# ToyotaResearchInstitute/conex

Measured on AMD Instinct MI355X. Metric: Newton KKT-solves/sec (assemble+factor+solve), 1000x(20x20) PSD blocks, fp64, higher is better.
Workload: dtype f64

## Files before the change

conex_amd/csrc/dense_elim.hip.h:

```cpp
#pragma once
#include "device_utils.h"

namespace cxk {

__device__ __forceinline__ void SqrtAndInverse(double d, double& root, double& inv) {
  const double r0 = __builtin_amdgcn_rsq(d);
  double g = d * r0, h = 0.5 * r0;
  double e = fma(-h, g, 0.5);
  g = fma(g, e, g);
  h = fma(h, e, h);
  e = fma(-h, g, 0.5);
  g = fma(g, e, g);
  h = fma(h, e, h);
  const double res = fma(-g, g, d);
  root = fma(res, h, g);
  inv = h + h;
}

template <int LEN, int C0, int C1, int BASE>
struct DppColumns {
  static __device__ __forceinline__ void run(double (&a)[LEN], double w, double v) {
    if constexpr (C0 < C1) {
      asm("v_fmac_f64_dpp %0, %1, %2 row_newbcast:%3 row_mask:0xf bank_mask:0xf"
          : "+v"(a[C0])
          : "v"(w), "v"(v), "n"(C0 - BASE));
      DppColumns<LEN, C0 + 1, C1, BASE>::run(a, w, v);
    }
  }
};

__device__ __forceinline__ void DppOperandFence(double& x, double& y, double& z) {
  asm("s_nop 1" : "+v"(x), "+v"(y), "+v"(z));
}


template <int NSMAX, int SMAX, int J, int C, int LEN>
__device__ __forceinline__ void ElimFmac(double (&a)[LEN], double x0, double x1) {
  if constexpr (C < 16) {
    asm volatile("v_fmac_f64_dpp %0, %1, -%2 row_newbcast:%3 row_mask:0xf bank_mask:0xf"
                 : "+v"(a[C])
                 : "v"(x0), "v"(a[J]), "n"(C));
  } else if constexpr (NSMAX == 16) {
    asm volatile("v_fmac_f64_dpp %0, %1, -%1 row_newbcast:%2 row_mask:0xf bank_mask:0xf"
                 : "+v"(a[C])
                 : "v"(a[J]), "n"(C - 16));
  } else {
    asm volatile("v_fmac_f64_dpp %0, %1, -%2 row_newbcast:%3 row_mask:0xf bank_mask:0xf"
                 : "+v"(a[C])
                 : "v"(x1), "v"(a[J]), "n"(C - 16));
  }
}

template <int NSMAX, int SMAX, int J, int P0, int CNT, int N, int LEN>
__device__ __forceinline__ void ElimIssue(double (&a)[LEN], double x0, double x1) {
  if constexpr (CNT > 0 && P0 < N) {
    ElimFmac<NSMAX, SMAX, J, J + 1 + P0>(a, x0, x1);
    ElimIssue<NSMAX, SMAX, J, P0 + 1, CNT - 1, N>(a, x0, x1);
  }
}

__device__ __forceinline__ int OpaqueLane(int lane) {
  int z;
  asm volatile("s_mov_b32 %0, 0" : "=s"(z));
  return lane + z;
}

template <int J>
__device__ __forceinline__ double ElimPivotColumn(double v, int lz, unsigned long long& m, double& s0, double& s1) {
  typedef unsigned u2 __attribute__((ext_vector_type(2)));
  __builtin_amdgcn_sched_barrier(0);
  m = __builtin_amdgcn_ballot_w64(lz == J);
  asm volatile("" : : "s"(m));
  __builtin_amdgcn_sched_barrier(0);
  double c0, c1;
  asm volatile("v_mov_b64 %0, %2\n\tv_mov_b64 %1, %2" : "=&v"(c0), "=&v"(c1) : "v"(v));
  __builtin_amdgcn_sched_barrier(0);
  const double d = ReadLane(v, J);
  __builtin_amdgcn_sched_barrier(0);
  const u2 l = __builtin_amdgcn_permlane16_swap(__double2loint(c0), __double2loint(c1), false, false);
  const u2 h = __builtin_amdgcn_permlane16_swap(__double2hiint(c0), __double2hiint(c1), false, false);
  s0 = __hiloint2double(h.x, l.x);
  s1 = __hiloint2double(h.y, l.y);
  __builtin_amdgcn_sched_barrier(0);
  return d;
}

template <int NSMAX, int SMAX, int J, int NRHS = 1, bool CHECK = true>
struct ElimSteps {
  static constexpr int LEN = NSMAX + SMAX + NRHS, RB = NSMAX + SMAX;
  static __device__ __forceinline__ void run(double (&a)[LEN], int lane, bool& bad, int ns) {
    if constexpr (J == 0 && NSMAX > 0) {
      if constexpr (kPipelined) {
        unsigned long long m;
        double s0, s1;
        const int lz = OpaqueLane(lane);
        const double d = ElimPivotColumn<0>(a[0], lz, m, s0, s1);
        if constexpr (CHECK) bad |= !(d > 0.0);
        double root, inv;
        SqrtAndInverse(d, root, inv);
        step(a, lane, bad, root, inv, ns, lz, m, s0, s1);
      } else {
        const double d = ReadLane(a[0], 0);
        if constexpr (CHECK) bad |= !(d > 0.0);
        double root, inv;
        SqrtAndInverse(d, root, inv);
        step(a, lane, bad, root, inv, ns);
      }
    }
  }
  static constexpr bool kPipelined = NSMAX + SMAX > 16 && NSMAX + SMAX <= 32;
  static __device__ __forceinline__ void step(double (&a)[LEN], int lane, bool& bad, double root, double inv, int ns,
                                              int lz = 0, unsigned long long m = 0, double s0 = 0.0, double s1 = 0.0) {
    if constexpr (kPipelined && J < NSMAX) {
      if (J >= ns) return;
      constexpr int N = NSMAX + SMAX - J - 1;
      const double x0 = s0 * inv, x1 = s1 * inv, t = a[J] * inv;
      __builtin_amdgcn_sched_barrier(0);
      a[J] = __builtin_amdgcn_inverse_ballot_w64(m) ? root : t;
      __builtin_amdgcn_sched_barrier(0);
      if constexpr (NSMAX == 16 && J + 1 >= 16 && N > 0) asm volatile("s_nop 1");
      ElimIssue<NSMAX, SMAX, J, 0, 1, N>(a, x0, x1);
      double root1 = 1.0, inv1 = 1.0, t0 = 0.0, t1 = 0.0;
      unsigned long long m1 = 0;
      if constexpr (J + 1 < NSMAX) {
        const double d1 = ElimPivotColumn<J + 1>(a[J + 1], lz, m1, t0, t1);
        if constexpr (CHECK) bad |= !(d1 > 0.0);
#define CXK_ELIM_FILL(P0, CNT)                      \
  __builtin_amdgcn_sched_barrier(0);                \
  ElimIssue<NSMAX, SMAX, J, P0, CNT, N>(a, x0, x1); \
  __builtin_amdgcn_sched_barrier(0)
        const double r0 = __builtin_amdgcn_rsq(d1);
        CXK_ELIM_FILL(1, 2);
        double g = d1 * r0, hh = 0.5 * r0;
        CXK_ELIM_FILL(3, 2);
        double e = fma(-hh, g, 0.5);
        CXK_ELIM_FILL(5, 2);
        g = fma(g, e, g);
        hh = fma(hh, e, hh);
        CXK_ELIM_FILL(7, 2);
        e = fma(-hh, g, 0.5);
        CXK_ELIM_FILL(9, 2);
        g = fma(g, e, g);
        hh = fma(hh, e, hh);
        CXK_ELIM_FILL(11, 2);
        const double res = fma(-g, g, d1);
        inv1 = hh + hh;
        CXK_ELIM_FILL(13, 2);
        root1 = fma(res, hh, g);
        CXK_ELIM_FILL(15, 64);
#undef CXK_ELIM_FILL
        asm volatile("" : : "v"(root1), "v"(inv1));
      } else {
        ElimIssue<NSMAX, SMAX, J, 1, 64, N>(a, x0, x1);
        __builtin_amdgcn_sched_barrier(0);
      }
#pragma unroll
      for (int q = 0; q < NRHS; q++) {
        const double yj = ReadLane(a[RB + q], J) * inv;
        if (lane > J)
          a[RB + q] = fma(-yj, a[J], a[RB + q]);
        else if (lane == J)
          a[RB + q] = yj;
      }
      ElimSteps<NSMAX, SMAX, J + 1, NRHS, CHECK>::step(a, lane, bad, root1, inv1, ns, lz, m1, t0, t1);
    } else if constexpr (J < NSMAX) {
      if (J >= ns) return;
      a[J] = (lane == J) ? root : a[J] * inv;
      double root1 = 1.0, inv1 = 1.0;
      auto next_pivot = [&]() {
        if constexpr (J + 1 < NSMAX) {
          const double d1 = ReadLane(a[J + 1], J + 1);
          if constexpr (CHECK) bad |= !(d1 > 0.0);
          SqrtAndInverse(d1, root1, inv1);
        }
      };
      if constexpr (NSMAX + SMAX <= 16) {
        double naj = -a[J];
        double dummy = 0.0;
        DppOperandFence(dummy, naj, a[J]);
        DppColumns<LEN, J + 1, (J + 2 < NSMAX + SMAX ? J + 2 : NSMAX + SMAX), 0>::run(a, a[J], naj);
        next_pivot();
        DppColumns<LEN, J + 2, NSMAX + SMAX, 0>::run(a, a[J], naj);
      } else {
        if constexpr (J + 1 < NSMAX + SMAX) a[J + 1] = fma(-ReadLane(a[J], J + 1), a[J], a[J + 1]);
        next_pivot();
#pragma unroll
        for (int c = J + 2; c < NSMAX + SMAX; c++) a[c] = fma(-ReadLane(a[J], c), a[J], a[c]);
      }
#pragma unroll
      for (int q = 0; q < NRHS; q++) {
        const double yj = ReadLane(a[RB + q], J) * inv;
        if (lane > J)
          a[RB + q] = fma(-yj, a[J], a[RB + q]);
        else if (lane == J)
          a[RB + q] = yj;
      }
      ElimSteps<NSMAX, SMAX, J + 1, NRHS, CHECK>::step(a, lane, bad, root1, inv1, ns);
    }
  }
};

}
```

conex_amd/csrc/tree_fused.hip:

```cpp
#include <hip/hip_runtime.h>
#include <hip/hip_ext.h>

#include <type_traits>

#include "tree_supernode.hip.h"
#include "kernels_kkt_top.hip.h"
#include "tree_fused.h"

namespace cxk {

constexpr int kFusedSpinLimit = 1 << 18;

#ifdef CXK_FUSED_STAMPS
constexpr int kFusedStampWaves = 8192;
__device__ long long g_fused_tree_stamp[kFusedStampWaves * 16];
#define FT_STAMP(i) ft_stamp[i] = __builtin_amdgcn_s_memrealtime()
#define FT_COUNT(i, v) ft_stamp[i] = (v)
#define FT_STAMP_DECL long long ft_stamp[16] = {0, 0, 0, 0, 0, 0, 0, 0, 0, 0, 0, 0, 0, 0, 0, 0}
#define FT_STAMP_FLUSH(level)                                                              \
  do {                                                                                     \
    if ((threadIdx.x & 63) == 0 && blockIdx.x < kFusedStampWaves) {                        \
      ft_stamp[15] = (level);                                                              \
      for (int i_ = 0; i_ < 16; i_++) g_fused_tree_stamp[blockIdx.x * 16 + i_] = ft_stamp[i_]; \
    }                                                                                      \
  } while (0)
#else
#define FT_STAMP(i) do { } while (0)
#define FT_COUNT(i, v) do { } while (0)
#define FT_STAMP_DECL do { } while (0)
#define FT_STAMP_FLUSH(level) do { } while (0)
#endif

__device__ __forceinline__ double LoadAgent(const double* p) {
  return __hip_atomic_load(p, __ATOMIC_RELAXED, __HIP_MEMORY_SCOPE_AGENT);
}
__device__ __forceinline__ void StoreAgent(double* p, double v) {
  __hip_atomic_store(p, v, __ATOMIC_RELAXED, __HIP_MEMORY_SCOPE_AGENT);
}
__device__ __forceinline__ bool IsSentinel(double v) {
  return (unsigned long long)__double_as_longlong(v) == kFusedSentinel;
}
__device__ __forceinline__ double SentinelValue() { return __longlong_as_double((long long)kFusedSentinel); }
__device__ __forceinline__ int64_t Join64(int lo, int hi) { return ((int64_t)hi << 32) | (uint32_t)lo; }

__device__ __forceinline__ void SleepUnits(int units) {
  for (; units >= 32; units -= 32) __builtin_amdgcn_s_sleep(32);
  for (; units >= 4; units -= 4) __builtin_amdgcn_s_sleep(4);
}

__device__ __forceinline__ void ReportTimeout(const FusedTreeArgs& A) {
  if ((threadIdx.x & 63) == 0) {
    atomicExch(A.fail + 1, A.tag);
    __hip_atomic_store(A.host_flag, 1.0, __ATOMIC_RELAXED, __HIP_MEMORY_SCOPE_SYSTEM);
  }
}

template <int NC, int PRW>
struct FusedImg {
  unsigned off[NC];
  unsigned aw, bi, o0, sl;
  int pd[PRW];
  unsigned pk[PRW];
};
struct FusedNoImg {};

constexpr int FusedRounds(int smax, int nrhs) { return (smax * (smax + 1) / 2 + nrhs * smax + 63) / 64; }
template <int NA, int SA, int NB, int SB, int NRHS>
struct FusedImgOf {
  static constexpr FusedImgLayout kLy = FusedImgLayoutOf(NA, SA, NB, SB);
  static constexpr int kRa = FusedRounds(SA, NRHS), kRb = FusedRounds(SB, NRHS);
  static constexpr int kRounds = kRa > kRb ? (kRa > 1 ? kRa : 1) : (kRb > 1 ? kRb : 1);
  using type = FusedImg<kLy.nc, kRounds>;
  static_assert(kLy.nc % 4 == 0 && NA + SA < kLy.rows && NB + SB < kLy.rows, "rows of four-word groups, one spare row");
  static __device__ __forceinline__ type Load(const FusedTreeArgs& A, int pos) {
    type I;
    const int lane = threadIdx.x & 63;
    const unsigned* im = A.img + (size_t)pos * kLy.stride;
    const int row = lane < kLy.rows - 1 ? lane : kLy.rows - 1;
    const uint4* po = reinterpret_cast<const uint4*>(im + row * kLy.nc);
#pragma unroll
    for (int q = 0; q < kLy.nc / 4; q++) {
      const uint4 v = po[q];
      I.off[4 * q] = v.x;
      I.off[4 * q + 1] = v.y;
      I.off[4 * q + 2] = v.z;
      I.off[4 * q + 3] = v.w;
    }
    const uint4 l = *reinterpret_cast<const uint4*>(im + kLy.l_at + 4 * row);
    I.aw = l.x;
    I.bi = l.y;
    I.o0 = l.z;
    I.sl = l.w;
#pragma unroll
    for (int r = 0; r < kRounds; r++) {
      const int t = lane + 64 * r;
      const uint2 u = *reinterpret_cast<const uint2*>(im + kLy.u_at + 2 * (t < kLy.ul ? t : 0));
      I.pd[r] = (int)u.x;
      I.pk[r] = u.y;
    }
    return I;
  }
};

template <int J>
__device__ __forceinline__ void FmacRowBcast(double& acc, double w, double v) {
  asm("v_fmac_f64_dpp %0, %1, %2 row_newbcast:%3 row_mask:0xf bank_mask:0xf" : "+v"(acc) : "v"(w), "v"(v), "n"(J));
}

template <int NSMAX, int SMAX, bool UP_ONLY = false, bool FROM_X = false, int NRHS = 1, class IMG = FusedNoImg>
__device__ __forceinline__ void FusedSupernode(const FusedTreeArgs& A, const int w, double* __restrict__ my, const IMG& I = IMG{}) {
  static_assert(NSMAX + SMAX <= 64, "one lane per panel row");
  constexpr bool IMAGED = !std::is_same<IMG, FusedNoImg>::value;
  static_assert(IMAGED == (!FROM_X && NSMAX <= 32), "two-row frames that load from the Schur blocks: the image");
  static_assert(NRHS == 1 || (NRHS == 3 && !UP_ONLY && !FROM_X && NSMAX <= 32), "three right-hand sides: the one-launch sweep of a single GPU");
  constexpr int RB = NSMAX + SMAX, MMAX = NRHS > 1 ? 4 : kFastSlots, MFMAX = MMAX, XMAX = kFusedExtraSlots;
  constexpr int RL = FusedRhsLane(NSMAX, SMAX);
  constexpr bool ROWRHS = RL >= 0 && !UP_ONLY && !FROM_X;
  constexpr int NCOL = ROWRHS ? 0 : NRHS;
  constexpr int NVMAX = SMAX * (SMAX + 1) / 2 + NRHS * SMAX;
  constexpr int PR = (NVMAX + 63) / 64;
  const int lane = threadIdx.x & 63;
  FT_STAMP_DECL;
  FT_STAMP(0);
  FT_COUNT(10, __builtin_amdgcn_s_getreg((31 << 11) | 4));
  FT_COUNT(11, __builtin_amdgcn_s_getreg((31 << 11) | 20));
  const SnRec R = DecodeRec(w);
  FT_STAMP(1);
  auto f = [&](int i) { return __builtin_amdgcn_readlane(w, 32 + i); };
  const int ns = R.ns, s = R.nsep;
  const bool is_row = lane < ns;
  const int sc = lane - NSMAX;
  const bool is_sep = sc >= 0 && sc < s;
  double* base = A.slab + R.diag_off;
  const unsigned rel = (unsigned)(R.offd_off - R.diag_off);
  unsigned o0, st;
  int lim;
  if constexpr (IMAGED) {
    o0 = I.o0;
    st = I.sl & 0xffffu;
    lim = (int)(I.sl >> 16);
  } else {
    o0 = is_row ? (unsigned)lane : (is_sep ? rel + (unsigned)(sc * ns) : 0u);
    st = is_row ? (unsigned)ns : 1u;
    lim = is_row ? lane + 1 : (is_sep ? ns : 0);
  }
  const int gen = A.gen;
  double* handG = A.hand + (int64_t)gen * A.hand_stride;
  double* handO = A.hand + (int64_t)(gen ^ 1) * A.hand_stride;
  double* ysG = A.ysig + (int64_t)gen * A.ysig_stride;
  double* ysO = A.ysig + (int64_t)(gen ^ 1) * A.ysig_stride;
  double* handT = A.hand + (int64_t)A.tgen * A.hand_stride;
  double* handTO = A.hand + (int64_t)(A.tgen ^ 1) * A.hand_stride;
  double* ysT = A.ysig + (int64_t)A.tgen * A.ysig_stride;
  double* ysTO = A.ysig + (int64_t)(A.tgen ^ 1) * A.ysig_stride;
  const int pub_beg = __builtin_amdgcn_readlane(w, 23);
  const int npairs = s * (s + 1) / 2, nv = npairs + NRHS * s;

  double a[NSMAX + SMAX + NCOL];
  double rv[NRHS];
  double fwx = 0.0;
  double awv, aqv;
  double rb;
  int pd[PR > 0 ? PR : 1], prd[PR > 0 ? PR : 1];
  bool pdt[PR > 0 ? PR : 1];
  pd[0] = prd[0] = 0;
  pdt[0] = false;
  if constexpr (IMAGED) {
    const char* gb = reinterpret_cast<const char*>(A.G);
#pragma unroll
    for (int j = 0; j < NSMAX; j++) a[j] = *reinterpret_cast<const double*>(gb + I.off[j]);
    awv = A.AWc[I.aw];
    aqv = A.AQcc[I.aw];
    rb = A.b[I.bi];
#pragma unroll
    for (int r = 0; r < PR; r++) {
      const unsigned pk = ROWRHS ? I.pk[r] : I.pk[r] >> 16;
      pd[r] = I.pd[r];
      prd[r] = (SMAX + NRHS) * (int)(pk & 255u) + (int)((pk >> 8) & 127u);
      pdt[r] = (int)I.pk[r] < 0;
    }
  } else {
  const double* Gk = A.G + (FROM_X ? 0 : Join64(f(0), f(1)));
  const int64_t roff = FROM_X ? 0 : Join64(f(2), f(3));
  const int M = f(4);
  const int q = is_row ? lane : (is_sep ? ns + sc : 0);
  const int mypr = (__builtin_amdgcn_ds_bpermute(4 * (32 + 6 + (q >> 2)), w) >> (8 * (q & 3))) & 255;
  const int myp = mypr == 255 ? 0 : mypr;
  const int has_fill = FROM_X ? 0 : f(5);
  if constexpr (FROM_X) {
    const int64_t xsb = Join64(f(0), f(1));
    const double* xd = A.x + xsb;
    const unsigned tri = (unsigned)(ns * (ns + 1) / 2);
#pragma unroll
    for (int j = 0; j < NSMAX; j++) {
      const unsigned dj = (unsigned)(j * ns - j * (j - 1) / 2);
      const unsigned idx = is_row ? dj + (unsigned)(lane - j) : tri + (unsigned)(sc * ns + j);
      a[j] = xd[(j < lim) ? idx : 0u];
    }
  } else {
    const char* gb = reinterpret_cast<const char*>(Gk);
    const unsigned myp8 = 8u * (unsigned)myp;
#pragma unroll
    for (int j = 0; j < NSMAX; j++) {
      const unsigned pj = (unsigned)((f(6 + (j >> 2)) >> (8 * (j & 3))) & 255);
      const unsigned pj8 = 8u * (pj == 255u ? 0u : pj);
      const unsigned hi8 = myp8 > pj8 ? myp8 : pj8, lo8 = myp8 > pj8 ? pj8 : myp8;
      a[j] = *reinterpret_cast<const double*>(gb + (__umul24(lo8, (unsigned)M) + hi8));
    }
    if (has_fill) {
#pragma unroll
      for (int j = 0; j < NSMAX; j++) {
        const unsigned pj = (unsigned)((f(6 + (j >> 2)) >> (8 * (j & 3))) & 255);
        a[j] = (mypr == 255 || pj == 255u) ? 0.0 : a[j];
      }
    }
  }
  const int pr = is_row ? myp : (f(6) & 255);
  if constexpr (FROM_X) {
    const int64_t xv = A.n_xs + f(2) + (is_row ? lane : 0);
    awv = A.x[xv];
    aqv = A.x[xv + A.n_xv];
    fwx = A.x[xv + 2 * (int64_t)A.n_xv];
  } else {
    awv = A.AWc[roff + pr];
    aqv = A.AQcc[roff + pr];
  }
  rb = A.b[R.start + (is_row ? lane : 0)];
#pragma unroll
  for (int r = 0; r < PR; r++) {
    const int t = lane + 64 * r;
    const int tq = (NRHS > 1 && t >= npairs + s && s > 0) ? (t - npairs) / s : 0;
    const int tk = t - tq * s;
    pdt[r] = tq > 0;
    pd[r] = A.pub[pub_beg + (t < nv ? tk : 0)] + tq * (int)A.fwd_stride;
    int k = 0, rem = t < npairs ? t : 0;
    while (rem >= s - k && k < s) {
      rem -= s - k;
      k++;
    }
    const int kk = t < npairs ? k : tk - npairs, cc = t < npairs ? k + rem : SMAX + tq;
    if (ROWRHS && t >= npairs)
      prd[r] = (SMAX + NRHS) * (RL + (t < nv ? tq : 0)) + (t < nv ? kk : 0);
    else
      prd[r] = (SMAX + NRHS) * (NSMAX + (t < nv ? kk : 0)) + (t < nv ? cc : 0);
  }
  }
  const int ntg = R.tg_end - R.tg_beg;
  int ploc0 = 0, ploc1 = 0;
  if (ntg > 0) {
    ploc0 = A.tg_reg[R.tg_beg + (lane < ntg ? lane : 0)];
    if (ntg > 64) ploc1 = A.tg_reg[R.tg_beg + (lane + 64 < ntg ? lane + 64 : 0)];
  }
  const int xt_beg = f(24), nxt = FROM_X ? 0 : f(25), mx = f(26), rbase = f(27), mr = FROM_X ? 0 : f(28);
  const int64_t xbase = Join64(f(29), f(30));
  int xloc0 = 0, xloc1 = 0;
  double gx0[XMAX], gx1[XMAX];
#pragma unroll
  for (int i = 0; i < XMAX; i++) gx0[i] = gx1[i] = 0.0;
  if (nxt > 0) {
    const int mxl = mx > 0 ? mx - 1 : 0;
    {
      const int ts = lane < nxt ? lane : 0;
      xloc0 = A.xreg[xt_beg + ts];
      long long xs[XMAX];
#pragma unroll
      for (int i = 0; i < XMAX; i++) xs[i] = A.xsrc[xbase + (int64_t)ts * mx + (i < mx ? i : mxl)];
#pragma unroll
      for (int i = 0; i < XMAX; i++) {
        const double v = A.G[xs[i] >= 0 ? xs[i] : 0];
        gx0[i] = (i < mx && xs[i] >= 0 && lane < nxt) ? v : 0.0;
      }
    }
    if (nxt > 64) {
      const int ts = lane + 64 < nxt ? lane + 64 : 0;
      xloc1 = A.xreg[xt_beg + ts];
      long long xs[XMAX];
#pragma unroll
      for (int i = 0; i < XMAX; i++) xs[i] = A.xsrc[xbase + (int64_t)ts * mx + (i < mx ? i : mxl)];
#pragma unroll
      for (int i = 0; i < XMAX; i++) {
        const double v = A.G[xs[i] >= 0 ? xs[i] : 0];
        gx1[i] = (i < mx && xs[i] >= 0 && lane + 64 < nxt) ? v : 0.0;
      }
    }
  }
#pragma unroll
  for (int j = 0; j < NSMAX; j++) a[j] = 0.0 + a[j];
  awv = 0.0 + awv;
  aqv = 0.0 + aqv;
  if (mr > 0) {
    const int mrl = mr - 1;
    long long rs[XMAX];
#pragma unroll
    for (int i = 0; i < XMAX; i++) rs[i] = A.rsrc[rbase + (is_row ? lane : 0) * mr + (i < mr ? i : mrl)];
    double ax[XMAX], qx[XMAX];
#pragma unroll
    for (int i = 0; i < XMAX; i++) {
      ax[i] = A.AWc[rs[i] >= 0 ? rs[i] : 0];
      qx[i] = A.AQcc[rs[i] >= 0 ? rs[i] : 0];
    }
    if (rs[0] >= 0) {
      awv = 0.0;
      aqv = 0.0;
    }
#pragma unroll
    for (int i = 0; i < XMAX; i++)
      if (i < mr && rs[i] >= 0) {
        awv += ax[i];
        aqv += qx[i];
      }
    for (int c0 = XMAX; c0 < mr; c0 += XMAX) {
#pragma unroll
      for (int i = 0; i < XMAX; i++) rs[i] = A.rsrc[rbase + (is_row ? lane : 0) * mr + (c0 + i < mr ? c0 + i : mrl)];
#pragma unroll
      for (int i = 0; i < XMAX; i++) {
        ax[i] = A.AWc[rs[i] >= 0 ? rs[i] : 0];
        qx[i] = A.AQcc[rs[i] >= 0 ? rs[i] : 0];
      }
#pragma unroll
      for (int i = 0; i < XMAX; i++)
        if (c0 + i < mr && rs[i] >= 0) {
          awv += ax[i];
          aqv += qx[i];
        }
    }
  }
  if constexpr (NRHS == 1) {
    if (A.comb)
      rb = A.cb * rb + A.cq * aqv + A.cw * awv;
    else
      rb = A.k * (rb * A.bs + aqv * A.cs) - 2 * awv;
  }
  if constexpr (FROM_X) rb -= fwx;
  if constexpr (!IMAGED) {
#pragma unroll
    for (int j = 0; j < NSMAX; j++) a[j] = (j < lim) ? a[j] : 0.0;
#pragma unroll
    for (int j = 0; j < NSMAX; j++)
      if (j >= ns && lane == j) a[j] = 1.0;
  }
#pragma unroll
  for (int c = 0; c < SMAX; c++) a[NSMAX + c] = 0.0;
  rv[0] = is_row ? (NRHS == 1 ? rb : rb * A.bs) : 0.0;
  if constexpr (NRHS == 3) {
    rv[1] = is_row ? aqv * A.cs : 0.0;
    rv[2] = is_row ? awv : 0.0;
  }
  FT_STAMP(2);

  const bool pulls = ntg > 0 || R.mf > 0;
  if (nxt > 0 || ntg > 0) {
#pragma unroll
    for (int j = 0; j < NSMAX; j++) my[64 * j + lane] = a[j];
    WaveSync();
    if (nxt > 0) {
      if (lane < nxt) {
        double acc = my[xloc0];
#pragma unroll
        for (int i = 0; i < XMAX; i++) acc += gx0[i];
        my[xloc0] = acc;
      }
      if (lane + 64 < nxt) {
        double acc = my[xloc1];
#pragma unroll
        for (int i = 0; i < XMAX; i++) acc += gx1[i];
        my[xloc1] = acc;
      }
      for (int c0 = XMAX; c0 < mx; c0 += XMAX)
        for (int half = 0; half < 2 && 64 * half < nxt; half++) {
          const int t = lane + 64 * half;
          const int ts = t < nxt ? t : 0;
          long long xs[XMAX];
          double gv[XMAX];
#pragma unroll
          for (int i = 0; i < XMAX; i++) xs[i] = A.xsrc[xbase + (int64_t)ts * mx + (c0 + i < mx ? c0 + i : mx - 1)];
#pragma unroll
          for (int i = 0; i < XMAX; i++) gv[i] = A.G[xs[i] >= 0 ? xs[i] : 0];
          const int xloc = half ? xloc1 : xloc0;
          double acc = my[xloc];
#pragma unroll
          for (int i = 0; i < XMAX; i++) acc += (c0 + i < mx && xs[i] >= 0) ? gv[i] : 0.0;
          if (t < nxt) my[xloc] = acc;
        }
      WaveSync();
    }
  }
  if (pulls) {
    double pv0[MMAX], pv1[MMAX], pb[MFMAX];
    double pbx[NRHS > 1 ? NRHS - 1 : 1][MFMAX];
    const double* srcx = handT + A.updb_base + A.fwd_stride + R.fbase + (is_row ? lane : 0) * R.mf;
    const double* src0 = handG + R.ubase + (int64_t)(lane < ntg ? lane : 0) * R.m;
    const double* src1 = handG + R.ubase + (int64_t)(lane + 64 < ntg ? lane + 64 : 0) * R.m;
    const double* srcb = handG + A.updb_base + R.fbase + (is_row ? lane : 0) * R.mf;
    const int span = R.m > R.mf ? R.m : R.mf;
    SleepUnits(f(31) * A.up_sleep);
    for (int sb0 = 0; sb0 < (span > 0 ? span : 1); sb0 += MMAX) {
    const int mleft = R.m - sb0, fleft = R.mf - sb0;
#pragma unroll
    for (int i = 0; i < MMAX; i++) pv1[i] = 0.0;
    if (ntg <= 64) {
      auto poll = [&](auto mmc) {
        constexpr int MM = decltype(mmc)::value;
        double p0[MM], pf[MM], q0[MM], qb[MM];
        double pfx[NRHS > 1 ? NRHS - 1 : 1][MM], qbx[NRHS > 1 ? NRHS - 1 : 1][MM];
        auto arrived = [&](const double (&v0)[MM], const double (&vb)[MM], const double (&vx)[NRHS > 1 ? NRHS - 1 : 1][MM]) {
          const bool is_tg = lane < ntg;
          bool pending = false;
#pragma unroll
          for (int i = 0; i < MM; i++) pending |= (i < mleft) & is_tg & IsSentinel(v0[i]);
#pragma unroll
          for (int i = 0; i < MM; i++) pending |= (i < fleft) & is_row & IsSentinel(vb[i]);
          if constexpr (NRHS > 1) {
#pragma unroll
            for (int q = 0; q < NRHS - 1; q++)
#pragma unroll
              for (int i = 0; i < MM; i++) pending |= (i < fleft) & is_row & IsSentinel(vx[q][i]);
          }
          return __ballot(pending) == 0;
        };
#define CXK_FUSED_ISSUE(V0, VB, VX)                                                      \
  do {                                                                                   \
    _Pragma("unroll") for (int i_ = 0; i_ < MM; i_++) V0[i_] = LoadAgent(src0 + (i_ < mleft ? sb0 + i_ : 0));   \
    _Pragma("unroll") for (int i_ = 0; i_ < MM; i_++) VB[i_] = LoadAgent(srcb + (i_ < fleft ? sb0 + i_ : 0)); \
    if constexpr (NRHS > 1) {                                                            \
      _Pragma("unroll") for (int q_ = 0; q_ < NRHS - 1; q_++)                            \
        _Pragma("unroll") for (int i_ = 0; i_ < MM; i_++)                                \
          VX[q_][i_] = LoadAgent(srcx + q_ * A.fwd_stride + (i_ < fleft ? sb0 + i_ : 0)); \
    }                                                                                    \
  } while (0)
        CXK_FUSED_ISSUE(p0, pf, pfx);
        for (int spin = 0;; spin++) {
          CXK_FUSED_ISSUE(q0, qb, qbx);
          if (arrived(p0, pf, pfx)) {
            FT_COUNT(12, 2 * spin);
            break;
          }
          CXK_FUSED_ISSUE(p0, pf, pfx);
          if (arrived(q0, qb, qbx) || 2 * spin >= kFusedSpinLimit) {
            if (2 * spin >= kFusedSpinLimit) ReportTimeout(A);
#pragma unroll
            for (int i = 0; i < MM; i++) p0[i] = q0[i];
#pragma unroll
            for (int i = 0; i < MM; i++) pf[i] = qb[i];
            if constexpr (NRHS > 1) {
#pragma unroll
              for (int q = 0; q < NRHS - 1; q++)
#pragma unroll
                for (int i = 0; i < MM; i++) pfx[q][i] = qbx[q][i];
            }
            FT_COUNT(12, 2 * spin + 1);
            break;
          }
        }
#undef CXK_FUSED_ISSUE
#pragma unroll
        for (int i = 0; i < MMAX; i++) pv0[i] = 0.0;
#pragma unroll
        for (int i = 0; i < MFMAX; i++) pb[i] = 0.0;
#pragma unroll
        for (int i = 0; i < MM; i++) pv0[i] = i < mleft ? p0[i] : 0.0;
#pragma unroll
        for (int i = 0; i < MM; i++) pb[i] = i < fleft ? pf[i] : 0.0;
        if constexpr (NRHS > 1) {
#pragma unroll
          for (int q = 0; q < NRHS - 1; q++) {
#pragma unroll
            for (int i = 0; i < MFMAX; i++) pbx[q][i] = 0.0;
#pragma unroll
            for (int i = 0; i < MM; i++) pbx[q][i] = i < fleft ? pfx[q][i] : 0.0;
          }
        }
      };
      if (mleft <= 4 && fleft <= 4)
        poll(std::integral_constant<int, 4>{});
      else
        poll(std::integral_constant<int, MMAX>{});
    } else {
      for (int spin = 0;; spin++) {
        bool pending = false;
#pragma unroll
        for (int i = 0; i < MMAX; i++) pv0[i] = pv1[i] = 0.0;
#pragma unroll
        for (int i = 0; i < MFMAX; i++) pb[i] = 0.0;
#pragma unroll
        for (int i = 0; i < MMAX; i++)
          if (i < mleft) {
            pv0[i] = LoadAgent(src0 + sb0 + i);
            pv1[i] = LoadAgent(src1 + sb0 + i);
          }
#pragma unroll
        for (int i = 0; i < MFMAX; i++)
          if (i < fleft) pb[i] = LoadAgent(srcb + sb0 + i);
        if constexpr (NRHS > 1) {
#pragma unroll
          for (int q = 0; q < NRHS - 1; q++)
#pragma unroll
            for (int i = 0; i < MFMAX; i++) {
              pbx[q][i] = i < fleft ? LoadAgent(srcx + q * A.fwd_stride + sb0 + i) : 0.0;
              pending |= is_row & IsSentinel(pbx[q][i]);
            }
        }
#pragma unroll
        for (int i = 0; i < MMAX; i++) {
          pending |= (lane < ntg) & IsSentinel(pv0[i]);
          pending |= (lane + 64 < ntg) & IsSentinel(pv1[i]);
        }
#pragma unroll
        for (int i = 0; i < MFMAX; i++) pending |= is_row & IsSentinel(pb[i]);
        if (__ballot(pending) == 0) {
          FT_COUNT(12, spin);
          break;
        }
        if (spin >= kFusedSpinLimit) {
          ReportTimeout(A);
          break;
        }
        __builtin_amdgcn_s_sleep(1);
      }
    }
    if (ntg > 0) {
      if (lane < ntg) {
        double acc = my[ploc0];
#pragma unroll
        for (int i = 0; i < MMAX; i++) acc -= pv0[i];
        my[ploc0] = acc;
      }
      if (lane + 64 < ntg) {
        double acc = my[ploc1];
#pragma unroll
        for (int i = 0; i < MMAX; i++) acc -= pv1[i];
        my[ploc1] = acc;
      }
      WaveSync();
    }
#pragma unroll
    for (int i = 0; i < MFMAX; i++) rv[0] -= is_row ? pb[i] : 0.0;
    if constexpr (NRHS > 1) {
#pragma unroll
      for (int q = 0; q < NRHS - 1; q++)
#pragma unroll
        for (int i = 0; i < MFMAX; i++) rv[1 + q] -= is_row ? pbx[q][i] : 0.0;
    }
    }
  }
  const bool imaged = nxt > 0 || ntg > 0;
  if (imaged) {
    if constexpr (ROWRHS) {
      if (lane < NSMAX) {
#pragma unroll
        for (int q = 0; q < NRHS; q++) my[64 * lane + RL + q] = rv[q];
      }
      WaveSync();
    }
#pragma unroll
    for (int j = 0; j < NSMAX; j++) a[j] = my[64 * j + lane];
    WaveSync();
  }
  if constexpr (ROWRHS) {
    if (!imaged) {
#pragma unroll
      for (int q = 0; q < NRHS; q++) my[64 * q + lane] = rv[q];
      WaveSync();
      if (lane >= RL && lane < RL + NRHS) {
#pragma unroll
        for (int j = 0; j < NSMAX; j++) a[j] = my[64 * (lane - RL) + j];
      }
      WaveSync();
    }
  } else {
#pragma unroll
    for (int q = 0; q < NRHS; q++) a[RB + q] = rv[q];
  }
  FT_STAMP(3);
  bool bad = false;
  if constexpr (NSMAX > 32) {
    static_assert(SMAX == 0, "the wide elimination has no separator rows");
    ElimWide<NSMAX, 0>::run(a, lane, ns, bad, [&](int j, double colj) {
      if (j < lim) base[o0 + j * st] = colj;
      my[65 * j + lane] = colj;
    });
  } else {
    ElimSteps<NSMAX, SMAX, 0, NCOL, !ROWRHS>::run(a, lane, bad, ns);
  }
  FT_STAMP(4);
  if (bad && lane == 0) atomicExch(A.fail + 1, A.tag);
  if constexpr (SMAX > 0) {
    if (s > 0) {
#pragma unroll
      for (int c = 0; c < SMAX; c++) my[(SMAX + NRHS) * lane + c] = a[NSMAX + c];
#pragma unroll
      for (int q = 0; q < NCOL; q++) my[(SMAX + NRHS) * lane + SMAX + q] = a[RB + q];
      WaveSync();
#pragma unroll
      for (int r = 0; r < PR; r++) {
        const double v = -my[prd[r]];
        if (lane + 64 * r < nv) StoreAgent((NRHS > 1 && pdt[r] ? handT : handG) + pd[r], v);
      }
      WaveSync();
    }
  }
  FT_STAMP(7);
  if constexpr (UP_ONLY) {
#pragma unroll
    for (int j = 0; j < NSMAX; j++)
      if (j < lim) base[o0 + j * st] = a[j];
    if (is_row) {
      A.y[R.start + lane] = a[NCOL > 0 ? RB : 0];
      A.AW[R.start + lane] = awv;
      A.AQc[R.start + lane] = aqv;
    }
    if constexpr (SMAX > 0) {
      if (s > 0) {
#pragma unroll
        for (int r = 0; r < PR; r++)
          if (lane + 64 * r < nv) StoreAgent(handO + pd[r], SentinelValue());
      }
    }
    return;
  }
  const int cnt = R.bs_end - R.bs_beg;
  const bool active = is_row;
  if constexpr (NSMAX <= 32) {
#pragma unroll
    for (int j = 0; j < NSMAX; j++) my[65 * j + lane] = a[j];
  }
  WaveSync();
  if (cnt > 0) {
#pragma unroll
    for (int j = 0; j < NSMAX; j++)
      if (j < lim) base[o0 + j * st] = a[j];
  }
  FT_STAMP(8);
  const int li = active ? lane : 0;
  double col[NSMAX];
#pragma unroll
  for (int k = 0; k < NSMAX; k++) col[k] = my[65 * li + k];
  double dg = my[66 * li];
  FT_STAMP(9);
  constexpr int QN = SMAX < 8 ? SMAX : 8;
  double bv[QN > 0 ? QN : 1], yv[QN > 0 ? QN : 1], Mb[QN > 0 ? QN : 1];
  double yvx[NRHS > 1 ? NRHS - 1 : 1][QN > 0 ? QN : 1];
  bv[0] = Mb[0] = 0.0;
#pragma unroll
  for (int qq = 0; qq < (QN > 0 ? QN : 1); qq++) {
    yv[qq] = 0.0;
#pragma unroll
    for (int q = 0; q < (NRHS > 1 ? NRHS - 1 : 1); q++) yvx[q][qq] = 0.0;
  }
  if constexpr (QN > 0) {
#pragma unroll
    for (int qq = 0; qq < QN; qq++) {
      const unsigned sw = qq < cnt ? (unsigned)R.sep[qq] : 0u;
      bv[qq] = my[65 * li + NSMAX + (int)(sw >> 26)];
    }
  }
#pragma unroll
  for (int k = 0; k < NSMAX; k++) col[k] = (active && k > lane && k < ns) ? col[k] : 0.0;
  dg = active ? dg : 1.0;
  double ub, ubx[NRHS > 1 ? NRHS - 1 : 1];
  ubx[0] = 0.0;
  if constexpr (ROWRHS) {
    ub = active ? my[65 * li + RL] : 0.0;
#pragma unroll
    for (int q = 0; q < NRHS - 1; q++) ubx[q] = active ? my[65 * li + RL + 1 + q] : 0.0;
  } else {
    ub = active ? a[NCOL > 0 ? RB : 0] : 0.0;
#pragma unroll
    for (int q = 0; q < NCOL - 1; q++) ubx[q] = active ? a[RB + 1 + q] : 0.0;
  }
  if constexpr (QN > 0) {
#pragma unroll
    for (int qq = 0; qq < QN; qq++) Mb[qq] = (qq < cnt && active) ? bv[qq] : 0.0;
  }
  {
    const double dinv = 1.0 / dg;
    const int lzb = OpaqueLane(lane);
#pragma unroll
    for (int k = NSMAX - 1; k >= 0; k--) {
      if (lzb == k) ub *= dinv;
      ub = fma(-col[k], ReadLane(ub, k), ub);
      if constexpr (NRHS > 1) {
#pragma unroll
        for (int q = 0; q < NRHS - 1; q++) {
          if (lzb == k) ubx[q] *= dinv;
          ubx[q] = fma(-col[k], ReadLane(ubx[q], k), ubx[q]);
        }
      }
      if constexpr (QN > 0) {
        if (cnt > 0) {
#pragma unroll
          for (int qq = 0; qq < QN; qq++) {
            if (lzb == k) Mb[qq] *= dinv;
            Mb[qq] = fma(-col[k], ReadLane(Mb[qq], k), Mb[qq]);
          }
        }
      }
    }
  }
  constexpr bool ROW0 = NSMAX <= 16 && QN > 0;
  double vsep = 0.0, vsepx[NRHS > 1 ? NRHS - 1 : 1];
#pragma unroll
  for (int q = 0; q < (NRHS > 1 ? NRHS - 1 : 1); q++) vsepx[q] = 0.0;
  if constexpr (ROW0) {
#pragma unroll
    for (int qq = 0; qq < QN; qq++) {
      Mb[qq] = -Mb[qq];
      asm volatile("" : "+v"(Mb[qq]));
    }
  }
  if constexpr (QN > 0) {
    if (cnt > 0) {
      const int sepw = __builtin_amdgcn_ds_bpermute(4 * (24 + (lane < 8 ? lane : 0)), w);
      const int sidx = lane < cnt ? (sepw & 0x3ffffff) : (R.sep[0] & 0x3ffffff);
      const double* src = ysG + sidx;
      double v;
      double vx[NRHS > 1 ? NRHS - 1 : 1];
      vx[0] = 0.0;
      for (int spin = 0;; spin++) {
        v = LoadAgent(src);
        bool pending = (lane < cnt) & IsSentinel(v);
        if constexpr (NRHS > 1) {
#pragma unroll
          for (int q = 0; q < NRHS - 1; q++) {
            vx[q] = LoadAgent(ysT + (int64_t)(1 + q) * A.y_stride + sidx);
            pending |= (lane < cnt) & IsSentinel(vx[q]);
          }
        }
        if (__ballot(pending) == 0) {
          FT_COUNT(14, spin);
          break;
        }
        if (spin >= kFusedSpinLimit) {
          ReportTimeout(A);
          break;
        }
        __builtin_amdgcn_s_sleep(1);
      }
      v = lane < cnt ? v : 0.0;
      if constexpr (NRHS > 1) {
#pragma unroll
        for (int q = 0; q < NRHS - 1; q++) vx[q] = lane < cnt ? vx[q] : 0.0;
      }
      if constexpr (ROW0) {
        vsep = v;
        if constexpr (NRHS > 1) {
#pragma unroll
          for (int q = 0; q < NRHS - 1; q++) vsepx[q] = vx[q];
        }
      } else {
#pragma unroll
        for (int qq = 0; qq < QN; qq++) yv[qq] = ReadLane(v, qq);
        if constexpr (NRHS > 1) {
#pragma unroll
          for (int q = 0; q < NRHS - 1; q++)
#pragma unroll
            for (int qq = 0; qq < QN; qq++) yvx[q][qq] = ReadLane(vx[q], qq);
        }
      }
    }
  }
  FT_STAMP(5);
  double accx[NRHS > 1 ? NRHS - 1 : 1];
  accx[0] = 0.0;
  double acc = ub;
  if constexpr (ROW0) {
    if constexpr (NRHS > 1) {
      static_assert(NRHS == 3, "two further right-hand sides");
      accx[0] = ubx[0];
      accx[1] = ubx[1];
      DppOperandFence(vsep, vsepx[0], vsepx[1]);
    } else {
      double d0 = 0.0, d1 = 0.0;
      DppOperandFence(vsep, d0, d1);
    }
    auto chain = [&](auto self, auto qc) {
      constexpr int qq = decltype(qc)::value;
      if constexpr (qq < QN) {
        FmacRowBcast<qq>(acc, vsep, Mb[qq]);
        if constexpr (NRHS > 1) {
          FmacRowBcast<qq>(accx[0], vsepx[0], Mb[qq]);
          FmacRowBcast<qq>(accx[1], vsepx[1], Mb[qq]);
        }
        self(self, std::integral_constant<int, qq + 1>{});
      }
    };
    chain(chain, std::integral_constant<int, 0>{});
  } else {
    if constexpr (NRHS > 1 && QN > 0) {
#pragma unroll
      for (int q = 0; q < NRHS - 1; q++) {
        accx[q] = ubx[q];
#pragma unroll
        for (int qq = 0; qq < QN; qq++) accx[q] = fma(-Mb[qq], yvx[q][qq], accx[q]);
      }
    } else if constexpr (NRHS > 1) {
#pragma unroll
      for (int q = 0; q < NRHS - 1; q++) accx[q] = ubx[q];
    }
    if constexpr (QN > 0) {
#pragma unroll
      for (int qq = 0; qq < QN; qq++) acc = fma(-Mb[qq], yv[qq], acc);
    }
  }
  if (active) StoreAgent(ysG + R.start + lane, acc);
  if constexpr (NRHS > 1) {
#pragma unroll
    for (int q = 0; q < NRHS - 1; q++)
      if (active) StoreAgent(ysT + (int64_t)(1 + q) * A.y_stride + R.start + lane, accx[q]);
  }
  FT_STAMP(6);
  if constexpr (ROWRHS) {
    if (__ballot(active && !(acc == acc)) != 0 && lane == 0) atomicExch(A.fail + 1, A.tag);
  }
  if (active) {
    if constexpr (NRHS == 3) {
      A.y3[R.start + lane] = acc;
      A.y3[A.y_stride + R.start + lane] = accx[0];
      A.y3[2 * A.y_stride + R.start + lane] = accx[1];
      A.y[R.start + lane] = accx[0] - acc;
      StoreAgent(ysTO + A.y_stride + R.start + lane, SentinelValue());
      StoreAgent(ysTO + 2 * A.y_stride + R.start + lane, SentinelValue());
    } else {
      A.y[R.start + lane] = acc;
    }
    A.AW[R.start + lane] = awv;
    A.AQc[R.start + lane] = aqv;
    StoreAgent(ysO + R.start + lane, SentinelValue());
  }
  if (NSMAX <= 32 && cnt == 0) {
#pragma unroll
    for (int j = 0; j < NSMAX; j++)
      if (j < lim) base[o0 + j * st] = a[j];
  }
  if constexpr (SMAX > 0) {
    if (s > 0) {
#pragma unroll
      for (int r = 0; r < PR; r++)
        if (lane + 64 * r < nv) StoreAgent((NRHS > 1 && pdt[r] ? handTO : handO) + pd[r], SentinelValue());
    }
  }
  FT_STAMP_FLUSH(f(31));
}

template <int NSMAX, int SMAX, int PHASE = 0>
__device__ __forceinline__ void FusedSolveSupernode(const FusedTreeArgs& A, const int w) {
  static_assert(NSMAX + SMAX <= 64, "one lane per panel row");
  constexpr int MFMAX = kFastSlots;
  constexpr int NVMAX = SMAX * (SMAX + 1) / 2 + SMAX;
  constexpr int PR = (NVMAX + 63) / 64;
  const int lane = threadIdx.x & 63;
  const SnRec R = DecodeRec(w);
  const int ns = R.ns, s = R.nsep;
  const bool is_row = lane < ns;
  const int sc = lane - NSMAX;
  const bool is_sep = sc >= 0 && sc < s;
  const double* base = A.slab + R.diag_off;
  const unsigned rel = (unsigned)(R.offd_off - R.diag_off);
  const unsigned o0 = is_row ? (unsigned)lane : (is_sep ? rel + (unsigned)(sc * ns) : 0u);
  const unsigned st = is_row ? (unsigned)ns : 1u;
  const int lim = is_row ? lane : (is_sep ? ns : 0);
  const int gen = A.gen;
  double* handG = A.hand + (int64_t)gen * A.hand_stride;
  double* handO = A.hand + (int64_t)(gen ^ 1) * A.hand_stride;
  double* ysG = A.ysig + (int64_t)gen * A.ysig_stride;
  double* ysO = A.ysig + (int64_t)(gen ^ 1) * A.ysig_stride;
  const int pub_beg = __builtin_amdgcn_readlane(w, 23);
  const int npairs = s * (s + 1) / 2, nv = npairs + s;
  const int cnt = R.bs_end - R.bs_beg;
  double a[NSMAX > 0 ? NSMAX : 1];
#pragma unroll
  for (int j = 0; j < NSMAX; j++) a[j] = base[(j < lim) ? o0 + j * st : 0u];
  double dg = base[is_row ? (unsigned)lane * (unsigned)(ns + 1) : 0u];
  const int p = R.start + (is_row ? lane : 0);
  double b;
  if (PHASE == 2 || A.form == 0) {
    b = A.y[p];
  } else {
    const double bp = A.b[p], aq = A.AQc[p], aw = A.AW[p];
    const double kk = (A.form == 1 && A.k_from) ? A.k_from[0] : A.k;
    b = A.form == 1 ? kk * (bp * A.bs + aq * A.cs) - 2 * aw : A.cb * bp + A.cq * aq + A.cw * aw;
  }
  const bool active = is_row;
  const double* D = A.slab + R.diag_off + (size_t)(active ? lane : 0) * ns;
  const double* B = A.slab + R.offd_off + (active ? lane : 0);
  double col[NSMAX];
#pragma unroll
  for (int k = 0; k < NSMAX; k++) col[k] = D[(active && k > lane && k < ns) ? k : 0];
  constexpr int QN = SMAX < 8 ? SMAX : 8;
  double bv[QN > 0 ? QN : 1], yv[QN > 0 ? QN : 1];
  bv[0] = yv[0] = 0.0;
#pragma unroll
  for (int qq = 0; qq < QN; qq++) {
    const unsigned sw = qq < cnt ? (unsigned)R.sep[qq] : 0u;
    const double* src = qq < cnt ? B + (size_t)(sw >> 26) * ns : D;
    bv[qq] = src[0];
  }
  int pdb = 0;
  if constexpr (SMAX > 0) pdb = A.pub[pub_beg + npairs + (is_sep ? sc : 0)];
  if constexpr (PHASE != 2) b = is_row ? b : 0.0;
  if (PHASE != 2 && R.mf > 0) {
    const double* srcb = handG + A.updb_base + R.fbase + (is_row ? lane : 0) * R.mf;
    for (int sb0 = 0; sb0 < R.mf; sb0 += MFMAX) {
      const int fleft = R.mf - sb0;
      double pb[MFMAX], qb[MFMAX];
      auto arrived = [&](const double (&vb)[MFMAX]) {
        bool pending = false;
#pragma unroll
        for (int i = 0; i < MFMAX; i++) pending |= (i < fleft) & is_row & IsSentinel(vb[i]);
        return __ballot(pending) == 0;
      };
#define CXK_FUSED_ISSUE(VB) \
  _Pragma("unroll") for (int i_ = 0; i_ < MFMAX; i_++) VB[i_] = LoadAgent(srcb + (i_ < fleft ? sb0 + i_ : 0))
      CXK_FUSED_ISSUE(pb);
      for (int spin = 0;; spin++) {
        CXK_FUSED_ISSUE(qb);
        if (arrived(pb)) break;
        CXK_FUSED_ISSUE(pb);
        if (arrived(qb) || 2 * spin >= kFusedSpinLimit) {
          if (2 * spin >= kFusedSpinLimit) ReportTimeout(A);
#pragma unroll
          for (int i = 0; i < MFMAX; i++) pb[i] = qb[i];
          break;
        }
      }
#undef CXK_FUSED_ISSUE
#pragma unroll
      for (int i = 0; i < MFMAX; i++) b -= (is_row && i < fleft) ? pb[i] : 0.0;
    }
  }
  if constexpr (PHASE != 2) {
#pragma unroll
  for (int j = 0; j < NSMAX; j++) a[j] = (j < lim) ? a[j] : 0.0;
  const double dinvf = is_row ? 1.0 / dg : 0.0;
  double dot = 0.0;
#pragma unroll
  for (int k = 0; k < NSMAX; k++) {
    if (lane == k) b *= dinvf;
    const double bk = ReadLane(b, k);
    if (is_sep)
      dot = fma(a[k], bk, dot);
    else
      b -= a[k] * bk;
  }
  if constexpr (SMAX > 0) {
    if (s > 0) {
      if (is_sep) StoreAgent(handG + pdb, dot);
    }
  }
  }
  if constexpr (PHASE == 1) {
    if (is_row) A.y[R.start + lane] = b;
  }
  if constexpr (PHASE != 1) {
  if constexpr (QN > 0) {
    if (cnt > 0) {
      const int sepw = __builtin_amdgcn_ds_bpermute(4 * (24 + (lane < 8 ? lane : 0)), w);
      const double* src = ysG + (lane < cnt ? (sepw & 0x3ffffff) : (R.sep[0] & 0x3ffffff));
      double v;
      for (int spin = 0;; spin++) {
        v = LoadAgent(src);
        if (__ballot(lane < cnt && IsSentinel(v)) == 0) break;
        if (spin >= kFusedSpinLimit) {
          ReportTimeout(A);
          break;
        }
        __builtin_amdgcn_s_sleep(1);
      }
#pragma unroll
      for (int qq = 0; qq < QN; qq++) yv[qq] = ReadLane(v, qq);
    }
  }
#pragma unroll
  for (int k = 0; k < NSMAX; k++) col[k] = (active && k > lane && k < ns) ? col[k] : 0.0;
  dg = active ? dg : 1.0;
  double acc = active ? b : 0.0;
  if constexpr (QN > 0) {
#pragma unroll
    for (int qq = 0; qq < QN; qq++) acc -= ((qq < cnt && active) ? bv[qq] : 0.0) * (qq < cnt ? yv[qq] : 0.0);
  }
  const double dinv = 1.0 / dg;
#pragma unroll
  for (int k = NSMAX - 1; k >= 0; k--) {
    if (lane == k) acc *= dinv;
    acc = fma(-col[k], ReadLane(acc, k), acc);
  }
  if (active) {
    StoreAgent(ysG + R.start + lane, acc);
    A.y[R.start + lane] = acc;
    StoreAgent(ysO + R.start + lane, SentinelValue());
  }
  }
  if constexpr (SMAX > 0 && PHASE != 2) {
    if (s > 0) {
#pragma unroll
      for (int r = 0; r < PR; r++) {
        const int t = lane + 64 * r;
        const int d = A.pub[pub_beg + (t < nv ? t : 0)];
        if (t < nv) StoreAgent(handO + d, SentinelValue());
      }
    }
  }
}

__device__ __forceinline__ void FusedScalars(const FusedTreeArgs& A) {
  const int lane = threadIdx.x & 63;
  double t0 = 0, t1 = 0;
#pragma unroll
  for (int v = 0; v < 4; v++) {
    double s0 = 0, s1 = 0;
    for (int i = 64 * v + lane; i < A.K; i += 256) {
      s0 += A.sc[2 * i];
      s1 += A.sc[2 * i + 1];
    }
    t0 += WaveSum(s0);
    t1 += WaveSum(s1);
  }
  if (lane == 0) {
    A.sys_sc[0] = t0;
    A.sys_sc[1] = t1;
    *A.fail = 0;
  }
}

template <int NA, int SA>
__device__ __forceinline__ bool FitsFrame(int ns, int s) { return ns <= NA && s <= SA; }

template <int NA, int SA, int NB, int SB, int MODE>
__global__ void __launch_bounds__(64, 2) tree_fused(FusedTreeArgs A) {
  extern __shared__ double lds[];
  const int pos = blockIdx.x;
  if (pos >= A.count) {
    FusedScalars(A);
    return;
  }
  const int w = A.rec[(size_t)pos * kFusedRecWords + (threadIdx.x & 63)];
  constexpr int NRHS = MODE == 2 ? 3 : 1;
  if constexpr (NA <= 32 && NB <= 32) {
    using Img = FusedImgOf<NA, SA, NB, SB, NRHS>;
    const typename Img::type I = Img::Load(A, pos);
    const int ns = __builtin_amdgcn_readlane(w, 1), s = __builtin_amdgcn_readlane(w, 2);
    if (NA == NB && SA == SB) {
      FusedSupernode<NA, SA, MODE == 1, false, NRHS>(A, w, lds, I);
    } else if (FitsFrame<NA, SA>(ns, s)) {
      FusedSupernode<NA, SA, MODE == 1, false, NRHS>(A, w, lds, I);
    } else {
      FusedSupernode<NB, SB, MODE == 1, false, NRHS>(A, w, lds, I);
    }
  } else {
    static_assert(NA == NB && SA == SB, "the wide instances are single-frame");
    FusedSupernode<NA, SA, MODE == 1, false, NRHS>(A, w, lds);
  }
}

__device__ __forceinline__ double WaitValue(const FusedTreeArgs& A, const double* p) {
  double v = LoadAgent(p);
  for (int spin = 0; IsSentinel(v); spin++) {
    if (spin >= kFusedSpinLimit) {
      atomicExch(A.fail + 1, A.tag);
      __hip_atomic_store(A.host_flag, 1.0, __ATOMIC_RELAXED, __HIP_MEMORY_SCOPE_SYSTEM);
      break;
    }
    __builtin_amdgcn_s_sleep(1);
    v = LoadAgent(p);
  }
  return v;
}

__device__ __forceinline__ void ShardPackItem(const FusedTreeArgs& A, int64_t item) {
  const double* handG = A.hand + (int64_t)A.gen * A.hand_stride;
  if (item < A.n_xs) {
    const GatherRec g = A.xg[item];
    double s = 0;
    if (g.first >= 0) s += A.G[g.first];
    for (int k = g.beg; k < g.beg + g.extra; k++) {
      const int64_t q = A.as_src[k];
      if (q >= 0) s += A.G[q];
    }
    const int t = A.xs_pt[item];
    if (t >= 0) {
      double u = 0;
      for (int q = A.pt_ptr[t]; q < A.pt_ptr[t + 1]; q++) u += WaitValue(A, handG + A.pt_src[q]);
      s -= u;
    }
    A.x[item] = s;
  } else if (item < A.n_xs + A.n_xv) {
    const int64_t j = item - A.n_xs;
    const ResidRec r = A.xr[j];
    double aw = 0, aq = 0;
    if (r.first >= 0) {
      aw += A.AWc[r.first];
      aq += A.AQcc[r.first];
    }
    for (int k = r.beg; k < r.beg + r.extra; k++) {
      aw += A.AWc[A.rs_src[k]];
      aq += A.AQcc[A.rs_src[k]];
    }
    double fw = 0;
    for (int q = A.pf_ptr[j]; q < A.pf_ptr[j + 1]; q++) fw += WaitValue(A, handG + A.updb_base + A.pf_src[q]);
    A.x[A.n_xs + j] = aw;
    A.x[A.n_xs + A.n_xv + j] = aq;
    A.x[A.n_xs + 2 * (int64_t)A.n_xv + j] = fw;
  }
}

__device__ __forceinline__ void ShardPackTail(const FusedTreeArgs& A) {
  FusedScalars(A);
  const int lane = threadIdx.x & 63;
  {
    const unsigned long long mine = lane < A.count_up ? (unsigned long long)((A.count_up - lane + 63) / 64) : 0ull;
    const unsigned long long want = A.done_target * mine;
    for (int spin = 0;; spin++) {
      const unsigned long long have = __hip_atomic_load(A.done + 16 * lane, __ATOMIC_RELAXED, __HIP_MEMORY_SCOPE_AGENT);
      if (__ballot(have < want) == 0) break;
      if (spin >= kFusedSpinLimit) {
        if (lane == 0) {
          atomicExch(A.fail + 1, A.tag);
          __hip_atomic_store(A.host_flag, 1.0, __ATOMIC_RELAXED, __HIP_MEMORY_SCOPE_SYSTEM);
        }
        break;
      }
      __builtin_amdgcn_s_sleep(2);
    }
  }
  if (lane == 0) {
    const int64_t o = A.n_xs + 3 * (int64_t)A.n_xv;
    const int f0 = __hip_atomic_load(A.fail, __ATOMIC_RELAXED, __HIP_MEMORY_SCOPE_AGENT);
    const int f1 = __hip_atomic_load(A.fail + 1, __ATOMIC_RELAXED, __HIP_MEMORY_SCOPE_AGENT);
    A.x[o] = A.sys_sc[0];
    A.x[o + 1] = A.sys_sc[1];
    const bool tagged = A.tag != 0 && f1 == A.tag;
    A.x[o + 2] = (f0 != 0 || tagged) ? 1.0 : 0.0;
    A.x[o + 3] = tagged && __hip_atomic_load(A.host_flag, __ATOMIC_RELAXED, __HIP_MEMORY_SCOPE_SYSTEM) != 0.0 ? 1.0 : 0.0;
  }
}

template <int NA, int SA, int NB, int SB>
__global__ void __launch_bounds__(64) tree_fused_shard_up(FusedTreeArgs A) {
  extern __shared__ double lds[];
  const int pos = blockIdx.x;
  if (pos < A.count_up) {
    const int w = A.rec[(size_t)pos * kFusedRecWords + (threadIdx.x & 63)];
    using Img = FusedImgOf<NA, SA, NB, SB, 1>;
    const typename Img::type I = Img::Load(A, pos);
// ... 169 lines not shown
```

Baseline: 25720.

## Use DPP row-broadcast back-substitution and issue sentinel stores before separator wait

```diff
diff --git a/conex_amd/csrc/dense_elim.hip.h b/conex_amd/csrc/dense_elim.hip.h
--- a/conex_amd/csrc/dense_elim.hip.h
+++ b/conex_amd/csrc/dense_elim.hip.h
@@ -31,6 +31,20 @@
 
 __device__ __forceinline__ void DppOperandFence(double& x, double& y, double& z) {
   asm("s_nop 1" : "+v"(x), "+v"(y), "+v"(z));
+}
+__device__ __forceinline__ void DppOperandFence(double& x) { asm("s_nop 1" : "+v"(x)); }
+template <int I = 0, int N>
+__device__ __forceinline__ void DppOperandFence(double (&x)[N]) {
+  if constexpr (N - I >= 4) {
+    asm("s_nop 1" : "+v"(x[I]), "+v"(x[I + 1]), "+v"(x[I + 2]), "+v"(x[I + 3]));
+    DppOperandFence<I + 4>(x);
+  } else if constexpr (N - I == 3) {
+    asm("s_nop 1" : "+v"(x[I]), "+v"(x[I + 1]), "+v"(x[I + 2]));
+  } else if constexpr (N - I == 2) {
+    asm("s_nop 1" : "+v"(x[I]), "+v"(x[I + 1]));
+  } else if constexpr (N - I == 1) {
+    asm("s_nop 1" : "+v"(x[I]));
+  }
 }
 
 
diff --git a/conex_amd/csrc/tree_fused.hip b/conex_amd/csrc/tree_fused.hip
--- a/conex_amd/csrc/tree_fused.hip
+++ b/conex_amd/csrc/tree_fused.hip
@@ -105,6 +105,10 @@
 template <int J>
 __device__ __forceinline__ void FmacRowBcast(double& acc, double w, double v) {
   asm("v_fmac_f64_dpp %0, %1, %2 row_newbcast:%3 row_mask:0xf bank_mask:0xf" : "+v"(acc) : "v"(w), "v"(v), "n"(J));
+}
+template <int J>
+__device__ __forceinline__ void FnmacRowBcast(double& acc, double w, double v) {
+  asm("v_fmac_f64_dpp %0, %1, -%2 row_newbcast:%3 row_mask:0xf bank_mask:0xf" : "+v"(acc) : "v"(w), "v"(v), "n"(J));
 }
 
 template <int NSMAX, int SMAX, bool UP_ONLY = false, bool FROM_X = false, int NRHS = 1, class IMG = FusedNoImg>
@@ -632,10 +636,13 @@
   }
   FT_STAMP(8);
   const int li = active ? lane : 0;
+  constexpr bool TUNED = !FROM_X;
+  double dg = 0.0;
+  if constexpr (TUNED) dg = my[66 * li];
   double col[NSMAX];
 #pragma unroll
   for (int k = 0; k < NSMAX; k++) col[k] = my[65 * li + k];
-  double dg = my[66 * li];
+  if constexpr (!TUNED) dg = my[66 * li];
   FT_STAMP(9);
   constexpr int QN = SMAX < 8 ? SMAX : 8;
   double bv[QN > 0 ? QN : 1], yv[QN > 0 ? QN : 1], Mb[QN > 0 ? QN : 1];
@@ -655,7 +662,7 @@
     }
   }
 #pragma unroll
-  for (int k = 0; k < NSMAX; k++) col[k] = (active && k > lane && k < ns) ? col[k] : 0.0;
+  for (int k = 0; k < NSMAX; k++) col[k] = (TUNED ? lane < (k < ns ? k : ns) : (active && k > lane && k < ns)) ? col[k] : 0.0;
   dg = active ? dg : 1.0;
   double ub, ubx[NRHS > 1 ? NRHS - 1 : 1];
   ubx[0] = 0.0;
@@ -675,8 +682,9 @@
   {
     const double dinv = 1.0 / dg;
     const int lzb = OpaqueLane(lane);
-#pragma unroll
-    for (int k = NSMAX - 1; k >= 0; k--) {
+    constexpr int KB = (NSMAX > 32 || !TUNED) ? 0 : (NSMAX < 16 ? NSMAX : 16);
+#pragma unroll
+    for (int k = NSMAX - 1; k >= KB; k--) {
       if (lzb == k) ub *= dinv;
       ub = fma(-col[k], ReadLane(ub, k), ub);
       if constexpr (NRHS > 1) {
@@ -696,6 +704,49 @@
         }
       }
     }
+    if constexpr (KB > 0) {
+      const double ds = lzb < KB ? dinv : 1.0;
+      auto sweep = [&](auto self, auto kc) {
+        constexpr int k = decltype(kc)::value;
+        {
+          double t = ub * ds;
+          if constexpr (NRHS > 1) {
+            static_assert(NRHS == 3, "two further right-hand sides");
+            double t1 = ubx[0] * ds, t2 = ubx[1] * ds;
+            DppOperandFence(t, t1, t2);
+            FnmacRowBcast<k>(ub, t, col[k]);
+            FnmacRowBcast<k>(ubx[0], t1, col[k]);
+            FnmacRowBcast<k>(ubx[1], t2, col[k]);
+          } else {
+            DppOperandFence(t);
+            FnmacRowBcast<k>(ub, t, col[k]);
+          }
+        }
+        if constexpr (QN > 0) {
+          if (cnt > 0) {
+            double tm[QN];
+#pragma unroll
+            for (int qq = 0; qq < QN; qq++) tm[qq] = Mb[qq] * ds;
+            DppOperandFence(tm);
+#pragma unroll
+            for (int qq = 0; qq < QN; qq++) FnmacRowBcast<k>(Mb[qq], tm[qq], col[k]);
+          }
+        }
+        if constexpr (k > 0) self(self, std::integral_constant<int, k - 1>{});
+      };
+      sweep(sweep, std::integral_constant<int, KB - 1>{});
+      ub *= ds;
+      if constexpr (NRHS > 1) {
+#pragma unroll
+        for (int q = 0; q < NRHS - 1; q++) ubx[q] *= ds;
+      }
+      if constexpr (QN > 0) {
+        if (cnt > 0) {
+#pragma unroll
+          for (int qq = 0; qq < QN; qq++) Mb[qq] *= ds;
+        }
+      }
+    }
   }
   constexpr bool ROW0 = NSMAX <= 16 && QN > 0;
   double vsep = 0.0, vsepx[NRHS > 1 ? NRHS - 1 : 1];
@@ -708,8 +759,33 @@
       asm volatile("" : "+v"(Mb[qq]));
     }
   }
+  auto row_stores = [&]() {
+    if (active) {
+      if constexpr (NRHS == 3) {
+        StoreAgent(ysTO + A.y_stride + R.start + lane, SentinelValue());
+        StoreAgent(ysTO + 2 * A.y_stride + R.start + lane, SentinelValue());
+      }
+      A.AW[R.start + lane] = awv;
+      A.AQc[R.start + lane] = aqv;
+      StoreAgent(ysO + R.start + lane, SentinelValue());
+    }
+  };
+  auto rearm_published = [&]() {
+    if constexpr (SMAX > 0) {
+      if (s > 0) {
+#pragma unroll
+        for (int r = 0; r < PR; r++)
+          if (lane + 64 * r < nv) StoreAgent((NRHS > 1 && pdt[r] ? handTO : handO) + pd[r], SentinelValue());
+      }
+    }
+  };
+  const bool stores_ahead = TUNED && QN > 0 && cnt > 0;
   if constexpr (QN > 0) {
     if (cnt > 0) {
+      if (stores_ahead) {
+        row_stores();
+        rearm_published();
+      }
       const int sepw = __builtin_amdgcn_ds_bpermute(4 * (24 + (lane < 8 ? lane : 0)), w);
       const int sidx = lane < cnt ? (sepw & 0x3ffffff) : (R.sep[0] & 0x3ffffff);
       const double* src = ysG + sidx;
@@ -818,27 +894,17 @@
       A.y3[A.y_stride + R.start + lane] = accx[0];
       A.y3[2 * A.y_stride + R.start + lane] = accx[1];
       A.y[R.start + lane] = accx[0] - acc;
-      StoreAgent(ysTO + A.y_stride + R.start + lane, SentinelValue());
-      StoreAgent(ysTO + 2 * A.y_stride + R.start + lane, SentinelValue());
     } else {
       A.y[R.start + lane] = acc;
     }
-    A.AW[R.start + lane] = awv;
-    A.AQc[R.start + lane] = aqv;
-    StoreAgent(ysO + R.start + lane, SentinelValue());
-  }
+  }
+  if (!stores_ahead) row_stores();
   if (NSMAX <= 32 && cnt == 0) {
 #pragma unroll
     for (int j = 0; j < NSMAX; j++)
       if (j < lim) base[o0 + j * st] = a[j];
   }
-  if constexpr (SMAX > 0) {
-    if (s > 0) {
-#pragma unroll
-      for (int r = 0; r < PR; r++)
-        if (lane + 64 * r < nv) StoreAgent((NRHS > 1 && pdt[r] ? handTO : handO) + pd[r], SentinelValue());
-    }
-  }
+  if (!stores_ahead) rearm_published();
   FT_STAMP_FLUSH(f(31));
 }
 
```

Result: no change. 25950, median of 6 (+0.9%).
